# carlobaldassi/GaussDCA.jl

Measured on AMD Instinct MI355X. Metric: end-to-end gDCA sec + achieved Cholesky TFLOP/s, N=500 M=50k q=21, higher is better.
Workload: dtype f64

## Files before the change

gaussdca.jl_amd/csrc/gdca_hamming_form.h:

```cpp
#pragma once

#if defined(__HIPCC__)
#define GDCA_FORM_HD __host__ __device__
#else
#define GDCA_FORM_HD
#endif

#define HAM_CAND_PER_TILE 64
#define HAM_FORM_MAX_DENSITY (0.5 * HAM_CAND_PER_TILE / 16384.0)

#define HAM_FORM_BOUND3_DENSITY 1e-3

#define HAM_T_DENSE 1.9e-3
#define HAM_CUT_TAIL 0.35
#define HAM_T_PAIR 0.7e-4
#define HAM_T_REFINE 1.3e-7
#define HAM_T_TILE 6.5e-3
#define HAM_T_ENTRY 1.6e-4
#define HAM_T_IMAGE 4.0e-5
#define HAM_T_FIXED 25.0

#define HAM_FORM_MIN_WORK 65536.0

static inline GDCA_FORM_HD double gdca_hamming_tiles(int M)
{
    const double Mt = (double)((M + 127) / 128);
    return 0.5 * Mt * (Mt + 1.0);
}

static inline GDCA_FORM_HD int gdca_hamming_consensus_gate(int N, int M)
{
    const int NW = (N + 31) / 32;
    return NW > 2 && gdca_hamming_tiles(M) * (double)NW >= HAM_FORM_MIN_WORK;
}

static inline GDCA_FORM_HD int gdca_hamming_pick_form(double cand3, double cand1, double pairs, int N, int M, int cut)
{
    if (!(pairs > 0.0)) return 0;
    const int NW = (N + 31) / 32;
    const double tiles = gdca_hamming_tiles(M), all = 0.5 * (double)M * (double)M;
    const double f3 = cand3 / pairs, f1 = cand1 / pairs;
    const int other = f3 < HAM_FORM_BOUND3_DENSITY ? 1 : 0;
    if (cand1 < 0.0 || f1 > HAM_FORM_MAX_DENSITY) return other;
    const double weff = (cut > 0 && cut < NW) ? (double)cut + HAM_CUT_TAIL * (double)(NW - cut) : (double)NW;
    const double E = (double)((NW + 7) / 8 * 8), pair = HAM_T_PAIR + (double)N * HAM_T_REFINE;
    const double cost_other = other ? tiles * weff * HAM_T_DENSE + f3 * all * pair : tiles * (double)NW * 1.5 * HAM_T_DENSE;
    const double cost_cons = tiles * (HAM_T_TILE + E * HAM_T_ENTRY) + f1 * all * pair + (double)M * E * HAM_T_IMAGE + HAM_T_FIXED;
    return cost_cons < cost_other ? 2 : other;
}
```

gaussdca.jl_amd/csrc/k_hamming_fp4.hip:

```cpp
#include <algorithm>

#include "gdca_internal.h"
#include "gdca_launch.h"

typedef int fp4x8_t __attribute__((ext_vector_type(8)));
typedef float f32x16_t __attribute__((ext_vector_type(16)));

#define F4_TILE 256
#define F4_KC 4
#define F4_ROW (F4_KC * 32 + 16)
#define F4_OP (F4_TILE * F4_ROW)
#define F4_LDS (4 * F4_OP)
#define F4_SEG 8

static inline int f4_entries(int NW) { return (NW + 2 * F4_KC - 1) / (2 * F4_KC) * (2 * F4_KC); }
static inline size_t f4_image_only_bytes(int N, int M)
{
    const size_t NW = (size_t)(N + 31) / 32, rows = ((size_t)M + F4_TILE - 1) / F4_TILE * F4_TILE;
    return rows * (size_t)f4_entries((int)NW) * 16;
}
size_t gdca_fp4_image_bytes(int N, int M)
{
    return f4_image_only_bytes(N, M) + (size_t)f4_entries((N + 31) / 32) * 32;
}

__device__ __forceinline__ uint32_t f4_spread8(uint32_t b)
{
    uint32_t x = b & 0xffu;
    x = (x | (x << 12)) & 0x000f000fu;
    x = (x | (x << 6)) & 0x03030303u;
    x = (x | (x << 3)) & 0x11111111u;
    return x;
}
__device__ __forceinline__ uint32_t f4_nibbles8(uint32_t differs, uint32_t valid)
{
    return ((f4_spread8(differs) << 3) | 0x22222222u) & (f4_spread8(valid) * 0xfu);
}
__device__ __forceinline__ uint32_t f4_signs8(uint32_t v)
{
    uint32_t x = (v >> 3) & 0x11111111u;
    x = (x | (x >> 3)) & 0x03030303u;
    x = (x | (x >> 6)) & 0x000f000fu;
    x = (x | (x >> 12)) & 0xffu;
    return x;
}

struct k_fp4_sigma_args {
    const uint32_t *hist;
    uint8_t *sigma;
    int N, NP;
};
template <int CAP>
__global__ __launch_bounds__(256) void k_fp4_sigma(const BatchArgs<k_fp4_sigma_args, CAP> B_)
{
    GDCA_MEMBER(B_);
    const uint32_t *__restrict__ hist = a_.hist;
    const int i = blockIdx.x * 256 + threadIdx.x;
    if (i >= a_.NP) return;
    uint32_t best = 0u, bz = 0u;
    if (i < a_.N) {
        const uint4 *h = reinterpret_cast<const uint4 *>(hist + (size_t)i * 32);
#pragma unroll
        for (int g = 0; g < 8; ++g) {
            const uint4 v = h[g];
            const uint32_t c[4] = {v.x, v.y, v.z, v.w};
#pragma unroll
// ... 16 lines not shown
template <int CAP>
__global__ __launch_bounds__(256) void k_fp4_image(const BatchArgs<k_fp4_image_args, CAP> B_)
{
    GDCA_MEMBER(B_);
    const int8_t *__restrict__ Z = a_.Z;
    const uint8_t *__restrict__ sigma = a_.sigma;
    uint4 *__restrict__ img = a_.img;
    const int N = a_.N, M = a_.M, E = a_.E;
    const long long g = (long long)blockIdx.x * 256 + threadIdx.x;
    if (g >= (long long)a_.rows * E) return;
    const int k = (int)(g / E), w = (int)(g - (long long)k * E);
    uint32_t diff = 0u, valid = 0u;
    const int nb = min(32, N - w * 32);
    if (k < M && nb > 0) {
        const int8_t *src = Z + (size_t)k * N + (size_t)w * 32;
        valid = nb == 32 ? 0xffffffffu : ((1u << nb) - 1u);
        if (nb == 32 && (N & 3) == 0 && (reinterpret_cast<uintptr_t>(Z) & 3) == 0) {
            const uint32_t *s4 = reinterpret_cast<const uint32_t *>(src), *g4 = reinterpret_cast<const uint32_t *>(sigma + w * 32);
#pragma unroll
            for (int j = 0; j < 8; ++j) {
                uint32_t x = (s4[j] & 0x1f1f1f1fu) ^ g4[j];
                x |= x >> 4;
                x |= x >> 2;
                x |= x >> 1;
                x &= 0x01010101u;
                diff |= (((x * 0x01020408u) >> 24) & 0xfu) << (4 * j);
            }
        } else {
            for (int b = 0; b < nb; ++b) diff |= (uint32_t)(((uint32_t)(uint8_t)src[b] & 31u) != (uint32_t)sigma[w * 32 + b]) << b;
        }
    }
    img[g] = make_uint4(f4_nibbles8(diff, valid), f4_nibbles8(diff >> 8, valid >> 8), f4_nibbles8(diff >> 16, valid >> 16), f4_nibbles8(diff >> 24, valid >> 24));
}

__device__ __forceinline__ void f4_tri_decode(int t, int Mt, int &I, int &J)
{
    const double b = 2.0 * Mt + 1.0;
    int i = (int)((b - sqrt(b * b - 8.0 * (double)t)) * 0.5);
    i = max(0, min(i, Mt - 1));
    auto start = [Mt](int r) { return (long long)r * Mt - (long long)r * (r - 1) / 2; };
    while (i > 0 && start(i) > t) --i;
    while (i < Mt - 1 && start(i + 1) <= t) ++i;
    I = i;
    J = i + (int)(t - start(i));
}

struct k_hamming_fp4_args {
    const unsigned char *img;
    int E, M, Mt, N;
    gdca_dev_scalars *sc;
    int2 *cand_list;
    unsigned cand_cap;
};
__shared__ unsigned f4_tile_n[2], f4_tile_base;
template <int CAP, bool ARES>
__global__ __launch_bounds__(1024) void k_hamming_fp4(const BatchArgs<k_hamming_fp4_args, CAP> B_)
{
    GDCA_MEMBER(B_);
    gdca_dev_scalars *__restrict__ sc = a_.sc;
    if (sc->ham_mode != 2) return;
    const int thresh = sc->thresh;
    if (thresh <= 0) return;
    const unsigned char *__restrict__ img = a_.img;
    const int E = a_.E, M = a_.M, Mt = a_.Mt;
    int2 *__restrict__ cand_list = a_.cand_list;
    const unsigned cand_cap = a_.cand_cap;
    extern __shared__ __attribute__((aligned(16))) unsigned char f4_lds[];

    const int I = (int)blockIdx.y, J0 = I + (int)blockIdx.x * F4_SEG;
    if (J0 >= Mt) return;
    const int J1 = min(Mt, J0 + F4_SEG);
    const int tid = threadIdx.x, lane = tid & 63, wv = tid >> 6, wr = wv & 3, wc = wv >> 2;
    const int l32 = lane & 31, lh = lane >> 5;
    if (tid == 0) {
        f4_tile_n[0] = 0u;
        f4_tile_n[1] = 0u;
    }
    const size_t rowbytes = (size_t)E * 16;
    const int nchunk = E / (2 * F4_KC);
    const int total = (J1 - J0) * nchunk;

    const int srow = tid >> 3, spc = tid & 7;
    const unsigned char *ga = img + ((size_t)I * F4_TILE + srow) * rowbytes + spc * 16;
    const unsigned char *gb0 = img + (size_t)srow * rowbytes + spc * 16;
    const size_t half = (size_t)128 * rowbytes, tilebytes = (size_t)F4_TILE * rowbytes;
    unsigned char *la = f4_lds + srow * F4_ROW + spc * 16;
    uint4 s0, s1, s2, s3;
    s0 = s1 = make_uint4(0u, 0u, 0u, 0u);
#define F4_LOAD_A(ch)                                                                     \
    do {                                                                                  \
        s0 = *reinterpret_cast<const uint4 *>(ga + (size_t)(ch) * (32 * F4_KC));          \
        s1 = *reinterpret_cast<const uint4 *>(ga + half + (size_t)(ch) * (32 * F4_KC));   \
    } while (0)
#define F4_LOAD_B(J, ch)                                                                                      \
    do {                                                                                                      \
        const unsigned char *g_ = gb0 + (size_t)(J) * tilebytes + (size_t)(ch) * (32 * F4_KC);                \
        s2 = *reinterpret_cast<const uint4 *>(g_);                                                            \
        s3 = *reinterpret_cast<const uint4 *>(g_ + half);                                                     \
    } while (0)
#define F4_STORE_A(region)                                                                \
    do {                                                                                  \
        unsigned char *d_ = la + (size_t)(region) * F4_OP;                                \
        *reinterpret_cast<uint4 *>(d_) = s0;                                              \
        *reinterpret_cast<uint4 *>(d_ + 128 * F4_ROW) = s1;                               \
    } while (0)
#define F4_STORE_B(buf)                                                                   \
    do {                                                                                  \
        unsigned char *d_ = la + (size_t)(2 + (buf)) * F4_OP;                             \
        *reinterpret_cast<uint4 *>(d_) = s2;                                              \
        *reinterpret_cast<uint4 *>(d_ + 128 * F4_ROW) = s3;                               \
    } while (0)

    f32x16_t acc[2][2];
#pragma unroll
    for (int i = 0; i < 2; ++i)
#pragma unroll
        for (int j = 0; j < 2; ++j)
#pragma unroll
            for (int e = 0; e < 16; ++e) acc[i][j][e] = 0.f;
    const int one = 0x7f7f7f7f;

    const unsigned char *abase = f4_lds + (wr * 64 + l32) * F4_ROW + lh * 16, *bbase = f4_lds + 2 * F4_OP + (wc * 64 + l32) * F4_ROW + lh * 16;
    const float limit = (float)(a_.N - 2 * thresh);

    if constexpr (ARES) {
        F4_LOAD_A(0);
        F4_STORE_A(0);
        if (nchunk > 1) {
            F4_LOAD_A(1);
            F4_STORE_A(1);
        }
    } else {
        F4_LOAD_A(0);
        F4_STORE_A(0);
    }
    F4_LOAD_B(J0, 0);
    F4_STORE_B(0);
    __syncthreads();
    int J = J0, ch = 0;
    for (int it = 0; it < total; ++it) {
        const int buf = it & 1;
        const bool more = it + 1 < total;
        const bool last = ch + 1 == nchunk;
        const int Jn = last ? J + 1 : J, chn = last ? 0 : ch + 1;
        if (more) {
            if constexpr (!ARES) F4_LOAD_A(chn);
            F4_LOAD_B(Jn, chn);
        }
        const unsigned char *As = abase + (size_t)(ARES ? ch : buf) * F4_OP, *Bs = bbase + (size_t)buf * F4_OP;
#pragma unroll 1
        for (int ks = 0; ks < F4_KC; ++ks) {
            fp4x8_t a[2], b[2];
#pragma unroll
            for (int i = 0; i < 2; ++i) {
                const uint4 x = *reinterpret_cast<const uint4 *>(As + i * 32 * F4_ROW + ks * 32);
                a[i] = (fp4x8_t){(int)x.x, (int)x.y, (int)x.z, (int)x.w, 0, 0, 0, 0};
            }
#pragma unroll
            for (int j = 0; j < 2; ++j) {
                const uint4 x = *reinterpret_cast<const uint4 *>(Bs + j * 32 * F4_ROW + ks * 32);
                b[j] = (fp4x8_t){(int)x.x, (int)x.y, (int)x.z, (int)x.w, 0, 0, 0, 0};
            }
#pragma unroll
            for (int i = 0; i < 2; ++i)
#pragma unroll
                for (int j = 0; j < 2; ++j)
                    acc[i][j] = __builtin_amdgcn_mfma_scale_f32_32x32x64_f8f6f4(a[i], b[j], acc[i][j], 4, 4, 0, one, 0, one);
        }
        if (more) {
            if constexpr (!ARES) F4_STORE_A(buf ^ 1);
            F4_STORE_B(buf ^ 1);
        }
        if (last) {
            const int slot_n = (J - J0) & 1;
            const bool diag = I == J;
            unsigned mine = 0;
            unsigned long long cand[2] = {0ull, 0ull};
            float mx = acc[0][0][0];
#pragma unroll
            for (int i = 0; i < 2; ++i)
#pragma unroll
                for (int j = 0; j < 2; ++j)
#pragma unroll
                    for (int e = 0; e < 16; ++e) mx = fmaxf(mx, acc[i][j][e]);
            if (mx > limit) {
#pragma unroll
                for (int i = 0; i < 2; ++i)
#pragma unroll
                    for (int j = 0; j < 2; ++j) {
                        const int gc = J * F4_TILE + wc * 64 + j * 32 + l32;
#pragma unroll
                        for (int e = 0; e < 16; ++e) {
                            const int gr = I * F4_TILE + wr * 64 + i * 32 + 8 * (e >> 2) + 4 * lh + (e & 3);
                            if (acc[i][j][e] > limit && gr < M && gc < M && (diag ? gr < gc : true)) {
                                cand[i] |= 1ull << (16 * j + e);
                                ++mine;
                            }
                        }
                    }
            }
#pragma unroll
            for (int i = 0; i < 2; ++i)
#pragma unroll
                for (int j = 0; j < 2; ++j)
#pragma unroll
                    for (int e = 0; e < 16; ++e) acc[i][j][e] = 0.f;
            const unsigned off = mine ? atomicAdd(&f4_tile_n[slot_n], mine) : 0u;
            __syncthreads();
            const unsigned ntile = f4_tile_n[slot_n];
            if (tid == 0) f4_tile_n[slot_n ^ 1] = 0u;
            if (ntile != 0u) {
                if (tid == 0) {
                    const unsigned long long base = atomicAdd(&sc->ham_ncand, (unsigned long long)ntile);
                    f4_tile_base = base > (unsigned long long)cand_cap ? cand_cap : (unsigned)base;
                }
                __syncthreads();
                unsigned slot = f4_tile_base + off;
#pragma unroll
                for (int i = 0; i < 2; ++i) {
                    unsigned long long c = cand[i];
                    while (c) {
                        const int bit = __builtin_ctzll(c), j = bit >> 4, e = bit & 15;
                        const int gr = I * F4_TILE + wr * 64 + i * 32 + 8 * (e >> 2) + 4 * lh + (e & 3);
                        const int gc = J * F4_TILE + wc * 64 + j * 32 + l32;
                        if (slot < cand_cap) cand_list[slot] = make_int2(gr, gc);
                        ++slot;
                        c &= c - 1;
                    }
                }
            }
        }
        J = Jn;
        ch = chn;
        __syncthreads();
    }
}

#define F4_PW 8
struct k_fp4_probe_args {
    const uint4 *img;
    int E, NW, M, Mt;
    gdca_dev_scalars *sc;
};
template <int CAP>
__global__ __launch_bounds__(256) void k_fp4_probe(const BatchArgs<k_fp4_probe_args, CAP> B_)
{
    GDCA_MEMBER(B_);
    const uint4 *__restrict__ img = a_.img;
    const int E = a_.E, NW = a_.NW, M = a_.M, Mt = a_.Mt;
    gdca_dev_scalars *sc = a_.sc;
    const int thresh = sc->thresh;
    if (thresh <= 0) return;
    __shared__ int total;
    __shared__ uint32_t bits[2][F4_PW][128];
    int I, J;
    f4_tri_decode((int)(((long long)blockIdx.x * ((long long)Mt * (Mt + 1) / 2)) / gridDim.x), Mt, I, J);
    const int tid = threadIdx.x, tx = tid & 15, ty = tid >> 4;
    if (tid == 0) total = 0;
    int D[8][8];
#pragma unroll
    for (int r = 0; r < 8; ++r)
#pragma unroll
        for (int c = 0; c < 8; ++c) D[r][c] = 0;
    const uint4 *mine = img + (size_t)((tid < 128 ? I : J) * 128 + (tid & 127)) * E;
    for (int w0 = 0; w0 < NW; w0 += F4_PW) {
        __syncthreads();
#pragma unroll
        for (int u = 0; u < F4_PW; ++u) {
            uint32_t b = 0u;
            if (w0 + u < NW) {
                const uint4 v = mine[w0 + u];
                b = f4_signs8(v.x) | (f4_signs8(v.y) << 8) | (f4_signs8(v.z) << 16) | (f4_signs8(v.w) << 24);
            }
            bits[tid >> 7][u][tid & 127] = b;
        }
        __syncthreads();
        const int wn = min(F4_PW, NW - w0);
        for (int u = 0; u < wn; ++u) {
            uint32_t a[8], b[8];
#pragma unroll
            for (int r = 0; r < 8; ++r) a[r] = bits[0][u][ty * 8 + r];
#pragma unroll
            for (int c = 0; c < 8; ++c) b[c] = bits[1][u][tx * 8 + c];
#pragma unroll
            for (int r = 0; r < 8; ++r)
#pragma unroll
                for (int c = 0; c < 8; ++c) D[r][c] += __builtin_popcount(a[r] ^ b[c]);
        }
    }
    int cand = 0;
#pragma unroll
    for (int r = 0; r < 8; ++r)
#pragma unroll
        for (int c = 0; c < 8; ++c) {
            const int gr = I * 128 + ty * 8 + r, gc = J * 128 + tx * 8 + c;
            cand += (gr < M) && (gc < M) && (gr != gc) && (D[r][c] < thresh);
        }
    if (cand) atomicAdd(&total, cand);
    __syncthreads();
    if (tid == 0 && total) atomicAdd(&sc->ham_cand2, total);
}

void gdca_launch_hamming_fp4_image(hipStream_t s, const int8_t *Z, const uint32_t *hist, void *img, int N, int M)
{
    const int NW = (N + 31) / 32, E = f4_entries(NW), rows = (M + F4_TILE - 1) / F4_TILE * F4_TILE;
    uint8_t *sigma = (uint8_t *)img + f4_image_only_bytes(N, M);
    gdca_launch<k_fp4_sigma_args, k_fp4_sigma<1>, k_fp4_sigma<GDCA_MAXB>>(dim3((unsigned)((32 * E + 255) / 256)), dim3(256), 0, s, k_fp4_sigma_args{hist, sigma, N, 32 * E});
    const long long items = (long long)rows * E;
    gdca_launch<k_fp4_image_args, k_fp4_image<1>, k_fp4_image<GDCA_MAXB>>(dim3((unsigned)((items + 255) / 256)), dim3(256), 0, s,
                                                                           k_fp4_image_args{Z, sigma, (uint4 *)img, N, M, E, rows});
}

void gdca_launch_hamming_fp4_probe(hipStream_t s, const void *img, int N, int M, int nprobe, gdca_dev_scalars *sc)
{
    const int NW = (N + 31) / 32, Mt = (M + 127) / 128;
    gdca_launch<k_fp4_probe_args, k_fp4_probe<1>, k_fp4_probe<GDCA_MAXB>>(dim3((unsigned)nprobe), dim3(256), 0, s,
                                                                           k_fp4_probe_args{(const uint4 *)img, f4_entries(NW), NW, M, Mt, sc});
}

void gdca_launch_hamming_fp4(hipStream_t s, const void *img, int N, int M, gdca_dev_scalars *sc, void *cand_list, unsigned cap)
{
    const int NW = (N + 31) / 32, E = f4_entries(NW), Mt = (M + F4_TILE - 1) / F4_TILE;
    const dim3 grid((unsigned)((Mt + F4_SEG - 1) / F4_SEG), (unsigned)Mt);
    const k_hamming_fp4_args a{(const unsigned char *)img, E, M, Mt, N, sc, (int2 *)cand_list, cap};
    if (E <= 4 * F4_KC)
        gdca_launch<k_hamming_fp4_args, k_hamming_fp4<1, true>, k_hamming_fp4<GDCA_MAXB, true>>(grid, dim3(1024), F4_LDS, s, a);
    else
        gdca_launch<k_hamming_fp4_args, k_hamming_fp4<1, false>, k_hamming_fp4<GDCA_MAXB, false>>(grid, dim3(1024), F4_LDS, s, a);
}
```

gaussdca.jl_amd/csrc/k_tally.hip:

```cpp
#include "gdca_internal.h"
#include "gdca_launch.h"
#include <cstdlib>

typedef unsigned long long u64;

#define PIK_THREADS 512
#define PIK_SLABS 4
struct k_pi_keep_args {
    const int8_t *Zt;
    const u64 *Wfix;
    u64 *Pifix;
    uint32_t *keep;
    int *keep_n;
    uint8_t *sigma;
    int N;
    int M;
    int q;
    gdca_dev_scalars *sc;
};
static inline k_pi_keep_args k_pi_keep_mk(const int8_t *Zt, const u64 *Wfix, u64 *Pifix, uint32_t *keep, int *keep_n, uint8_t *sigma, int N, int M, int q, gdca_dev_scalars *sc)
{
    return k_pi_keep_args{Zt, Wfix, Pifix, keep, keep_n, sigma, N, M, q, sc};
}
template <int CAP>
// ... 258 lines not shown
void gdca_launch_pi_finalize(hipStream_t s, const u64 *Pifix, int N, int q, int fix_shift, const double *Meff_dev,
                             double pc, double *Pi_true, double *Pi_pc, double *pi_max)
{
    const int n = N * (q - 1);
    (gdca_launch<k_pi_finalize_args, k_pi_finalize<1>, k_pi_finalize<GDCA_MAXB>>(dim3((n + 255) / 256), dim3(256), 0, s, k_pi_finalize_mk(Pifix, N, q, fix_shift, Meff_dev, pc, Pi_true, Pi_pc, pi_max)));
}

#define TALLY_THREADS 1024
#define TALLY_CHUNK 1024

struct k_pair_tally_args {
    const int8_t *Zc;
    const int8_t *Zt;
    const u64 *Wfix;
    int N;
    int M;
    int q;
    int fix_shift;
    const double *Meff_dev;
    double pc;
    const double *Pi_pc;
    int mode;
    double *out;
    size_t ld;
    const uint32_t *keep;
    const int *keep_n;
    const uint8_t *sigma;
    const u64 *Pifix;
};
static inline k_pair_tally_args k_pair_tally_mk(const int8_t *Zc, const int8_t *Zt, const u64 *Wfix, int N, int M, int q, int fix_shift, const double *Meff_dev, double pc, const double *Pi_pc, int mode, double *out, size_t ld,
                                                const uint32_t *keep, const int *keep_n, const uint8_t *sigma, const u64 *Pifix)
{
    return k_pair_tally_args{Zc, Zt, Wfix, N, M, q, fix_shift, Meff_dev, pc, Pi_pc, mode, out, ld, keep, keep_n, sigma, Pifix};
}
template <int CAP, int TJ, bool SKIP>
__global__ __launch_bounds__(TALLY_THREADS) void k_pair_tally(const BatchArgs<k_pair_tally_args, CAP> B_)
{
    GDCA_MEMBER(B_);
    const int8_t *__restrict__ Zc = a_.Zc;
    const int8_t *__restrict__ Zt = a_.Zt;
    const u64 *__restrict__ Wfix = a_.Wfix;
    int N = a_.N;
    int M = a_.M;
    int q = a_.q;
    int fix_shift = a_.fix_shift;
    const double *__restrict__ Meff_dev = a_.Meff_dev;
    double pc = a_.pc;
    const double *__restrict__ Pi_pc = a_.Pi_pc;
    int mode = a_.mode;
    double *__restrict__ out = a_.out;
    size_t ld = a_.ld;
    extern __shared__ __attribute__((aligned(16))) unsigned char smem[];
    const int s = q - 1;
    const int i = blockIdx.y;
    const int jblk = (blockIdx.x + blockIdx.y) % gridDim.x;
    const int j0 = jblk * TJ;
    if (j0 + TJ - 1 < i) return;

    const int NROW = SKIP ? q : s;
    const int CB = SKIP ? 0 : 1;
    const int RS = (SKIP ? q : s + 2) * TJ;
    u64 *hist = reinterpret_cast<u64 *>(smem);
    u64 *meta_s = hist + (size_t)NROW * RS;
    uint8_t *zs = reinterpret_cast<uint8_t *>(meta_s + TALLY_CHUNK);

    const int tid = threadIdx.x, lane = tid & 63, wv = tid >> 6;
    constexpr int SPI = 64 / TJ;
    constexpr int NWAVE = TALLY_THREADS / 64;
    constexpr int SEQ_PER_WAVE = TALLY_CHUNK / NWAVE;
    constexpr int NV = TJ / 16;
    static_assert(TALLY_CHUNK == TALLY_THREADS, "one staged sequence per thread");
    const int jl = lane % TJ, sub = lane / TJ;
    const u64 wmask = (1ull << 59) - 1;
    const unsigned qclamp = (unsigned)(SKIP ? q - 1 : s + 1);
    const int nk = SKIP ? a_.keep_n[i] : M;
    const uint32_t *__restrict__ keep_i = a_.keep + (size_t)i * M;

    for (int e = tid; e < NROW * RS; e += TALLY_THREADS) hist[e] = 0;

    const int8_t *Zblk = Zc + (size_t)jblk * M * TJ;
    uint4 z0 = make_uint4(0, 0, 0, 0), z1 = z0;
    u64 wf = 0;
    int8_t av = 0;
#define TALLY_FETCH(KC)                                                                       \
    do {                                                                                      \
        int k_ = (KC) + tid;                                                                  \
        k_ = k_ < nk ? k_ : nk - 1;              \
        if (SKIP) {                                                                           \
            const uint32_t e_ = keep_i[k_];                                                   \
            av = (int8_t)(e_ & 31u);                                                          \
            k_ = (int)(e_ >> 5);                                                              \
        }                                                                                     \
        const uint4 *src_ = reinterpret_cast<const uint4 *>(Zblk + (size_t)k_ * TJ);          \
        z0 = src_[0];                                                                         \
        if (NV > 1) z1 = src_[1];                                                             \
        if (!SKIP) av = Zt[(size_t)i * M + k_];                                               \
        wf = Wfix[k_];                                                                        \
    } while (0)
    if (nk > 0) TALLY_FETCH(0);
    for (int kc = 0; kc < nk; kc += TALLY_CHUNK) {
        __syncthreads();
        {
            reinterpret_cast<uint4 *>(zs + (size_t)tid * TJ)[0] = z0;
            if (NV > 1) reinterpret_cast<uint4 *>(zs + (size_t)tid * TJ)[1] = z1;
            const unsigned a = (unsigned)(uint8_t)av - 1u;
            const bool valid = (SKIP || a < (unsigned)s) && (kc + tid < nk);
            meta_s[tid] = valid ? (((u64)a << 59) | (wf & wmask)) : 0ull;
        }
        __syncthreads();
        if (kc + TALLY_CHUNK < nk) TALLY_FETCH(kc + TALLY_CHUNK);
        const int kw = wv * SEQ_PER_WAVE;
#pragma unroll 2
        for (int it = 0; it < SEQ_PER_WAVE / SPI; it += 4) {
            u64 m4[4];
            unsigned b4[4];
#pragma unroll
            for (int u = 0; u < 4; ++u) {
                const int kk = kw + (it + u) * SPI + sub;
                m4[u] = meta_s[kk];
                b4[u] = zs[kk * TJ + jl];
            }
#pragma unroll
            for (int u = 0; u < 4; ++u) {
                const unsigned a = (unsigned)(m4[u] >> 59);
                const unsigned b = min(b4[u] - (unsigned)(1 - CB), qclamp);
                const unsigned idx = __umul24(a, (unsigned)RS) + __umul24(b, (unsigned)TJ) + (unsigned)jl;
                atomicAdd(&hist[idx], m4[u] & wmask);
            }
        }
    }
    __syncthreads();
#undef TALLY_FETCH

    if (SKIP) {
        const int sg = (int)a_.sigma[i] - 1;
        const u64 *__restrict__ Pifix = a_.Pifix;
        if (sg < s) {
            for (int e = tid; e < s * TJ; e += TALLY_THREADS) {
                const int b = e / TJ, l = e - b * TJ;
                const int jj = j0 + l;
                if (jj >= N || jj < i) continue;
                u64 v = Pifix[(size_t)jj * 32 + b + 1];
                for (int a = 0; a < q; ++a)
                    if (a != sg) v -= hist[(size_t)a * RS + b * TJ + l];
                hist[(size_t)sg * RS + b * TJ + l] = v;
            }
        }
    }

    double *pi_i = reinterpret_cast<double *>(meta_s);
    double *pi_j = pi_i + 32;
    if (mode == 1) {
        for (int e = tid; e < s; e += TALLY_THREADS) pi_i[e] = Pi_pc[i * s + e];
        for (int e = tid; e < TJ * s; e += TALLY_THREADS) {
            const int jj = j0 + e / s;
            pi_j[e] = (jj < N) ? Pi_pc[jj * s + (e % s)] : 0.0;
        }
    }
    __syncthreads();
    const double Meff = *Meff_dev;
    const double pcq = pc / (double)q;
    const double off_add = pcq / (double)q;
    const int total = s * s * TJ;
    for (int e = tid; e < total; e += TALLY_THREADS) {
        const int a = e / (TJ * s), rem = e - a * (TJ * s);
        const int l = rem / s, b = rem - l * s;
        const int jj = j0 + l;
        if (jj >= N || jj < i) continue;
        const double pt = ldexp((double)hist[(size_t)a * RS + (b + CB) * TJ + l], -fix_shift) / Meff;
        double v = pt;
        if (mode == 1) {
            const double pij = (jj != i) ? ((1.0 - pc) * pt + off_add) : ((1.0 - pc) * pt + ((a == b) ? pcq : 0.0));
            v = pij - pi_i[a] * pi_j[rem];
        }
        out[(size_t)(jj * s + b) + (size_t)(i * s + a) * ld] = v;
    }
    for (int e = tid; e < total; e += TALLY_THREADS) {
        const int l = e / (s * s), rem = e - l * (s * s);
        const int b = rem / s, a = rem - b * s;
        const int jj = j0 + l;
        if (jj >= N || jj <= i) continue;
        const double pt = ldexp((double)hist[(size_t)a * RS + (b + CB) * TJ + l], -fix_shift) / Meff;
        double v = pt;
        if (mode == 1) {
            const double pij = (1.0 - pc) * pt + off_add;
            v = pij - pi_i[a] * pi_j[l * s + b];
        }
        out[(size_t)(i * s + a) + (size_t)(jj * s + b) * ld] = v;
    }
}

static size_t tally_lds_bytes(int s, int TJ, bool skip = false)
{
    const size_t hist = skip ? (size_t)(s + 1) * (s + 1) * TJ * 8 : (size_t)s * (s + 2) * TJ * 8;
    return hist + (size_t)TALLY_CHUNK * 8 + (size_t)TALLY_CHUNK * TJ;
}

int gdca_tally_tj(int q, int tj_wanted)
{
    if (tj_wanted == 32 && tally_lds_bytes(q - 1, 32) <= 160 * 1024) return 32;
    return 16;
}

bool gdca_tally_skip(int q, int TJ, int skip_wanted, int M)
{
    const size_t lds = 160 * 1024, full = tally_lds_bytes(q - 1, TJ), skip = tally_lds_bytes(q - 1, TJ, true);
    return skip_wanted && M <= (1 << 27) && skip <= lds && lds / skip >= lds / full;
}

void gdca_launch_pair_tally(hipStream_t st, const int8_t *Zc, const int8_t *Zt, const u64 *Wfix, int N, int M, int q,
                            int fix_shift, const double *Meff_dev, double pc, const double *Pi_pc, int mode,
                            double *out, size_t ld, int TJ, const uint32_t *keep, const int *keep_n, const uint8_t *sigma,
                            const u64 *Pifix)
{
    const int s = q - 1;
    const bool skip = keep != nullptr;
    const k_pair_tally_args a = k_pair_tally_mk(Zc, Zt, Wfix, N, M, q, fix_shift, Meff_dev, pc, Pi_pc, mode, out, ld, keep, keep_n, sigma, Pifix);
    const size_t lds = tally_lds_bytes(s, TJ, skip);
    if (TJ == 32) {
        if (skip)
            (gdca_launch<k_pair_tally_args, k_pair_tally<1, 32, true>, k_pair_tally<GDCA_MAXB, 32, true>>(dim3((N + 31) / 32, N), dim3(TALLY_THREADS), lds, st, a));
        else
            (gdca_launch<k_pair_tally_args, k_pair_tally<1, 32, false>, k_pair_tally<GDCA_MAXB, 32, false>>(dim3((N + 31) / 32, N), dim3(TALLY_THREADS), lds, st, a));
    } else {
        if (skip)
            (gdca_launch<k_pair_tally_args, k_pair_tally<1, 16, true>, k_pair_tally<GDCA_MAXB, 16, true>>(dim3((N + 15) / 16, N), dim3(TALLY_THREADS), lds, st, a));
        else
            (gdca_launch<k_pair_tally_args, k_pair_tally<1, 16, false>, k_pair_tally<GDCA_MAXB, 16, false>>(dim3((N + 15) / 16, N), dim3(TALLY_THREADS), lds, st, a));
    }
}

#define COV_ROWS_PER_THREAD 4
struct k_cov_from_pij_args {
    const double *Pij;
    const double *Pi_pc;
    int n;
    int q;
    double pc;
    double *out;
    size_t ld;
};
static inline k_cov_from_pij_args k_cov_from_pij_mk(const double *Pij, const double *Pi_pc, int n, int q, double pc, double *out, size_t ld)
{
    return k_cov_from_pij_args{Pij, Pi_pc, n, q, pc, out, ld};
}
template <int CAP>
__global__ __launch_bounds__(256) void k_cov_from_pij(const BatchArgs<k_cov_from_pij_args, CAP> B_)
{
    GDCA_MEMBER(B_);
    const double *__restrict__ Pij = a_.Pij;
    const double *__restrict__ Pi_pc = a_.Pi_pc;
    int n = a_.n;
    int q = a_.q;
    double pc = a_.pc;
    double *__restrict__ out = a_.out;
    size_t ld = a_.ld;
    const int s = q - 1;
    const int c = blockIdx.y;
    const int ic = c / s;
    const double pcq = pc / (double)q;
    const double off_add = pcq / (double)q;
    const double pi_c = Pi_pc[c];
    const double *__restrict__ src = Pij + (size_t)c * n;
    double *__restrict__ dst = out + (size_t)c * ld;
    const int r0 = blockIdx.x * (256 * COV_ROWS_PER_THREAD) + threadIdx.x;
    double pt[COV_ROWS_PER_THREAD], pr[COV_ROWS_PER_THREAD];
#pragma unroll
    for (int u = 0; u < COV_ROWS_PER_THREAD; ++u) {
        const int r = r0 + u * 256;
        pt[u] = r < n ? src[r] : 0.0;
        pr[u] = r < n ? Pi_pc[r] : 0.0;
    }
#pragma unroll
    for (int u = 0; u < COV_ROWS_PER_THREAD; ++u) {
        const int r = r0 + u * 256;
        if (r >= n) continue;
        const int jj = r / s, i = ic;
        const bool ab = r == c;
        const double pij = (jj != i) ? ((1.0 - pc) * pt[u] + off_add) : ((1.0 - pc) * pt[u] + (ab ? pcq : 0.0));
        dst[r] = pij - pi_c * pr[u];
    }
// ... 9 lines not shown
```

Baseline: 52.41.

## Restructure FP4 Hamming MFMA kernel: 512 threads, wider warp tiles, deeper pipelined loads

Rewrites the FP4 Hamming candidate kernel to use 512-thread blocks where each wave computes a 64x128 tile (2x4 MFMA accumulators). It loads through buffer resources, prefetches two chunks ahead, and schedules LDS reads against MFMAs with sched_group_barrier. It also remaps the grid to a 1D triangular walk enumeration with XCD-aware interleaving and defers candidate writes by one tile to overlap the global atomic. The cost-model constants for the consensus form are lowered to match, so the form picker will choose this path more often. This raises register pressure and adds complexity in the triple-buffered tile counters and the deferred-write synchronisation.

```diff
diff --git a/gaussdca.jl_amd/csrc/gdca_hamming_form.h b/gaussdca.jl_amd/csrc/gdca_hamming_form.h
--- a/gaussdca.jl_amd/csrc/gdca_hamming_form.h
+++ b/gaussdca.jl_amd/csrc/gdca_hamming_form.h
@@ -15,8 +15,8 @@
 #define HAM_CUT_TAIL 0.35
 #define HAM_T_PAIR 0.7e-4
 #define HAM_T_REFINE 1.3e-7
-#define HAM_T_TILE 6.5e-3
-#define HAM_T_ENTRY 1.6e-4
+#define HAM_T_TILE 4.8e-3
+#define HAM_T_ENTRY 1.2e-4
 #define HAM_T_IMAGE 4.0e-5
 #define HAM_T_FIXED 25.0
 
diff --git a/gaussdca.jl_amd/csrc/k_hamming_fp4.hip b/gaussdca.jl_amd/csrc/k_hamming_fp4.hip
--- a/gaussdca.jl_amd/csrc/k_hamming_fp4.hip
+++ b/gaussdca.jl_amd/csrc/k_hamming_fp4.hip
@@ -5,6 +5,8 @@
 
 typedef int fp4x8_t __attribute__((ext_vector_type(8)));
 typedef float f32x16_t __attribute__((ext_vector_type(16)));
+typedef unsigned u32x4_t __attribute__((ext_vector_type(4)));
+typedef float f32x2_t __attribute__((ext_vector_type(2)));
 
 #define F4_TILE 256
 #define F4_KC 4
@@ -12,6 +14,7 @@
 #define F4_OP (F4_TILE * F4_ROW)
 #define F4_LDS (4 * F4_OP)
 #define F4_SEG 8
+#define F4_THREADS 512
 
 static inline int f4_entries(int NW) { return (NW + 2 * F4_KC - 1) / (2 * F4_KC) * (2 * F4_KC); }
 static inline size_t f4_image_only_bytes(int N, int M)
@@ -134,9 +137,138 @@
     int2 *cand_list;
     unsigned cand_cap;
 };
-__shared__ unsigned f4_tile_n[2], f4_tile_base;
+__shared__ unsigned f4_tile_n[3], f4_tile_base;
+
+static inline __host__ __device__ unsigned f4_walks(int Mt)
+{
+    const unsigned nb = (unsigned)((Mt + F4_SEG - 1) / F4_SEG);
+    return (F4_SEG / 2) * (nb - 1) * nb + (unsigned)Mt;
+}
+
+__device__ __forceinline__ fp4x8_t f4_frag(const unsigned char *p)
+{
+    const uint4 x = *reinterpret_cast<const uint4 *>(p);
+    return (fp4x8_t){(int)x.x, (int)x.y, (int)x.z, (int)x.w, 0, 0, 0, 0};
+}
+template <bool FIRST, bool TWOSETS>
+__device__ __forceinline__ void f4_chunk(f32x16_t (&acc)[2][4], const unsigned char *As, const unsigned char *Bs)
+{
+    static_assert(F4_KC == 4, "the schedule below is written for four k steps");
+    const int one = 0x7f7f7f7f;
+    const f32x16_t zero = (f32x16_t)(0.f);
+    fp4x8_t a0[2], b0[4], a1[2], b1[4];
+    (void)a1, (void)b1;
+#define F4_READ(a, b, ks)                                                        \
+    do {                                                                         \
+        _Pragma("unroll") for (int i = 0; i < 2; ++i) a[i] = f4_frag(As + i * 32 * F4_ROW + (ks) * 32); \
+        _Pragma("unroll") for (int j = 0; j < 4; ++j) b[j] = f4_frag(Bs + j * 32 * F4_ROW + (ks) * 32); \
+    } while (0)
+#define F4_MUL(a, b, C)                                                          \
+    do {                                                                         \
+        _Pragma("unroll") for (int i = 0; i < 2; ++i)                            \
+            _Pragma("unroll") for (int j = 0; j < 4; ++j)                        \
+                acc[i][j] = __builtin_amdgcn_mfma_scale_f32_32x32x64_f8f6f4(a[i], b[j], C, 4, 4, 0, one, 0, one); \
+    } while (0)
+    if constexpr (TWOSETS) {
+        F4_READ(a0, b0, 0);
+        F4_READ(a1, b1, 1);
+        if constexpr (FIRST)
+            F4_MUL(a0, b0, zero);
+        else
+            F4_MUL(a0, b0, acc[i][j]);
+        F4_READ(a0, b0, 2);
+        F4_MUL(a1, b1, acc[i][j]);
+        F4_READ(a1, b1, 3);
+        F4_MUL(a0, b0, acc[i][j]);
+        F4_MUL(a1, b1, acc[i][j]);
+        __builtin_amdgcn_sched_group_barrier(0x100, 6, 0);
+#pragma unroll
+        for (int ks = 0; ks + 1 < F4_KC; ++ks)
+#pragma unroll
+            for (int m = 0; m < 8; ++m) {
+                __builtin_amdgcn_sched_group_barrier(0x008, 1, 0);
+                if (m < 6) __builtin_amdgcn_sched_group_barrier(0x100, 1, 0);
+            }
+        __builtin_amdgcn_sched_group_barrier(0x008, 8, 0);
+    } else {
+        F4_READ(a0, b0, 0);
+        if constexpr (FIRST)
+            F4_MUL(a0, b0, zero);
+        else
+            F4_MUL(a0, b0, acc[i][j]);
+#pragma unroll 1
+        for (int ks = 1; ks < F4_KC; ++ks) {
+            F4_READ(a0, b0, ks);
+            F4_MUL(a0, b0, acc[i][j]);
+        }
+    }
+#undef F4_READ
+#undef F4_MUL
+}
+
+__device__ __forceinline__ void f4_tile_candidates(const f32x16_t (&acc)[2][4], const float limit, const int I, const int J, const int M, const int wr,
+                                                   const int wc, const int l32, const int lh, const int slot_n, unsigned long long (&cand)[2],
+                                                   unsigned &off)
+{
+    unsigned mine = 0u;
+    cand[0] = cand[1] = 0ull;
+    const bool diag = I == J, edge = diag || (J + 1) * F4_TILE > M;
+    int rb = I * F4_TILE + wr * 64 + 4 * lh, cb = J * F4_TILE + wc * 128 + l32;
+    asm volatile("" : "+v"(rb), "+v"(cb));
+#pragma unroll
+    for (int i = 0; i < 2; ++i)
+#pragma unroll
+        for (int j = 0; j < 4; ++j) {
+            float mx = acc[i][j][0];
+#pragma unroll
+            for (int e = 1; e < 16; ++e) mx = __builtin_amdgcn_fmed3f(mx, acc[i][j][e], __builtin_inff());
+            if (mx > limit) {
+                unsigned m16 = 0u;
+#pragma unroll
+                for (int e = 14; e >= 0; e -= 2) {
+                    const f32x2_t d = (f32x2_t)(limit) - (f32x2_t){acc[i][j][e], acc[i][j][e + 1]};
+                    m16 = __builtin_amdgcn_alignbit(m16, __float_as_uint(d.y), 31u);
+                    m16 = __builtin_amdgcn_alignbit(m16, __float_as_uint(d.x), 31u);
+                }
+                if (edge) {
+                    const int gc = cb + j * 32;
+#pragma unroll
+                    for (int e = 0; e < 16; ++e) {
+                        const int gr = rb + i * 32 + 8 * (e >> 2) + (e & 3);
+                        if (!(gr < M && gc < M && (diag ? gr < gc : true))) m16 &= ~(1u << e);
+                    }
+                }
+                cand[i] |= (unsigned long long)m16 << (16 * j);
+                mine += (unsigned)__builtin_popcount(m16);
+            }
+        }
+    off = mine ? atomicAdd(&f4_tile_n[slot_n], mine) : 0u;
+}
+__device__ __forceinline__ unsigned f4_tile_count(const int tid, const int slot_n)
+{
+    const unsigned ntile = f4_tile_n[slot_n];
+    if (tid == 0) f4_tile_n[slot_n == 0 ? 2 : slot_n - 1] = 0u;
+    return (unsigned)__builtin_amdgcn_readfirstlane((int)ntile);
+}
+__device__ __forceinline__ void f4_tile_write(int2 *cand_list, const unsigned cand_cap, const int I, const int J, const int wr, const int wc, const int l32,
+                                              const int lh, const unsigned long long (&cand)[2], unsigned slot)
+{
+#pragma unroll
+    for (int i = 0; i < 2; ++i) {
+        unsigned long long c = cand[i];
+        while (c) {
+            const int bit = __builtin_ctzll(c), j = bit >> 4, e = bit & 15;
+            const int gr = I * F4_TILE + wr * 64 + i * 32 + 8 * (e >> 2) + 4 * lh + (e & 3);
+            const int gc = J * F4_TILE + wc * 128 + j * 32 + l32;
+            if (slot < cand_cap) cand_list[slot] = make_int2(gr, gc);
+            ++slot;
+            c &= c - 1;
+        }
+    }
+}
+
 template <int CAP, bool ARES>
-__global__ __launch_bounds__(1024) void k_hamming_fp4(const BatchArgs<k_hamming_fp4_args, CAP> B_)
+__global__ __launch_bounds__(F4_THREADS) void k_hamming_fp4(const BatchArgs<k_hamming_fp4_args, CAP> B_)
 {
     GDCA_MEMBER(B_);
     gdca_dev_scalars *__restrict__ sc = a_.sc;
@@ -149,173 +281,170 @@
     const unsigned cand_cap = a_.cand_cap;
     extern __shared__ __attribute__((aligned(16))) unsigned char f4_lds[];
 
-    const int I = (int)blockIdx.y, J0 = I + (int)blockIdx.x * F4_SEG;
-    if (J0 >= Mt) return;
-    const int J1 = min(Mt, J0 + F4_SEG);
+    int I, J0, J1;
+    {
+        const unsigned id = blockIdx.x, x = id & 7u, k = id >> 3;
+        const unsigned v = ((k >> 5) * 8u + x) * 32u + (k & 31u);
+        if (v >= f4_walks(Mt)) return;
+        int c = (int)((sqrtf((float)v + 1.f) - 1.f) * 0.5f);
+        c = max(c, 0);
+        while (c > 0 && (unsigned)((F4_SEG / 2) * c * (c + 1)) > v) --c;
+        while ((unsigned)((F4_SEG / 2) * (c + 1) * (c + 2)) <= v) ++c;
+        I = (int)(v - (unsigned)((F4_SEG / 2) * c * (c + 1)));
+        J0 = max(I, c * F4_SEG);
+        J1 = min(Mt, (c + 1) * F4_SEG);
+    }
+    if (I >= Mt || J0 >= J1) return;
     const int tid = threadIdx.x, lane = tid & 63, wv = tid >> 6, wr = wv & 3, wc = wv >> 2;
     const int l32 = lane & 31, lh = lane >> 5;
     if (tid == 0) {
         f4_tile_n[0] = 0u;
         f4_tile_n[1] = 0u;
+        f4_tile_n[2] = 0u;
     }
     const size_t rowbytes = (size_t)E * 16;
     const int nchunk = E / (2 * F4_KC);
     const int total = (J1 - J0) * nchunk;
 
     const int srow = tid >> 3, spc = tid & 7;
-    const unsigned char *ga = img + ((size_t)I * F4_TILE + srow) * rowbytes + spc * 16;
-    const unsigned char *gb0 = img + (size_t)srow * rowbytes + spc * 16;
-    const size_t half = (size_t)128 * rowbytes, tilebytes = (size_t)F4_TILE * rowbytes;
-    unsigned char *la = f4_lds + srow * F4_ROW + spc * 16;
-    uint4 s0, s1, s2, s3;
-    s0 = s1 = make_uint4(0u, 0u, 0u, 0u);
-#define F4_LOAD_A(ch)                                                                     \
-    do {                                                                                  \
-        s0 = *reinterpret_cast<const uint4 *>(ga + (size_t)(ch) * (32 * F4_KC));          \
-        s1 = *reinterpret_cast<const uint4 *>(ga + half + (size_t)(ch) * (32 * F4_KC));   \
+    const unsigned voff = (unsigned)srow * (unsigned)rowbytes + (unsigned)spc * 16u, quarter = 64u * (unsigned)rowbytes;
+    const size_t tilebytes = (size_t)F4_TILE * rowbytes;
+    const unsigned char *ga = img + (size_t)I * tilebytes;
+    const unsigned char *gn = img + (size_t)J0 * tilebytes;
+    int ldch = 0;
+    unsigned char *la = f4_lds + srow * F4_ROW + spc * 16, *lb = la + 2 * F4_OP;
+#define F4_LOAD(S, g, live)                                                                                                \
+    do {                                                                                                                \
+        const __amdgpu_buffer_rsrc_t r_ = __builtin_amdgcn_make_buffer_rsrc(const_cast<unsigned char *>(g), 0, (live) ? (int)tilebytes : 0, 0x00020000); \
+        S##0 = __builtin_amdgcn_raw_buffer_load_b128(r_, (int)voff, 0, 0);                                              \
+        S##1 = __builtin_amdgcn_raw_buffer_load_b128(r_, (int)voff, (int)quarter, 0);                                   \
+        S##2 = __builtin_amdgcn_raw_buffer_load_b128(r_, (int)voff, (int)(2u * quarter), 0);                            \
+        S##3 = __builtin_amdgcn_raw_buffer_load_b128(r_, (int)voff, (int)(3u * quarter), 0);                            \
     } while (0)
-#define F4_LOAD_B(J, ch)                                                                                      \
-    do {                                                                                                      \
-        const unsigned char *g_ = gb0 + (size_t)(J) * tilebytes + (size_t)(ch) * (32 * F4_KC);                \
-        s2 = *reinterpret_cast<const uint4 *>(g_);                                                            \
-        s3 = *reinterpret_cast<const uint4 *>(g_ + half);                                                     \
+#define F4_STORE(S, l, region)                                            \
+    do {                                                                  \
+        unsigned char *d_ = (l) + (region) * F4_OP;                       \
+        *reinterpret_cast<u32x4_t *>(d_) = S##0;                          \
+        *reinterpret_cast<u32x4_t *>(d_ + 64 * F4_ROW) = S##1;            \
+        *reinterpret_cast<u32x4_t *>(d_ + 128 * F4_ROW) = S##2;           \
+        *reinterpret_cast<u32x4_t *>(d_ + 192 * F4_ROW) = S##3;           \
     } while (0)
-#define F4_STORE_A(region)                                                                \
-    do {                                                                                  \
-        unsigned char *d_ = la + (size_t)(region) * F4_OP;                                \
-        *reinterpret_cast<uint4 *>(d_) = s0;                                              \
-        *reinterpret_cast<uint4 *>(d_ + 128 * F4_ROW) = s1;                               \
+#define F4_NEXT()                                                         \
+    do {                                                                  \
+        gn += 32 * F4_KC;                                                 \
+        if (++ldch == nchunk) {                                           \
+            ldch = 0;                                                     \
+            gn += tilebytes - (size_t)nchunk * (32 * F4_KC);              \
+        }                                                                 \
     } while (0)
-#define F4_STORE_B(buf)                                                                   \
-    do {                                                                                  \
-        unsigned char *d_ = la + (size_t)(2 + (buf)) * F4_OP;                             \
-        *reinterpret_cast<uint4 *>(d_) = s2;                                              \
-        *reinterpret_cast<uint4 *>(d_ + 128 * F4_ROW) = s3;                               \
-    } while (0)
-
-    f32x16_t acc[2][2];
-#pragma unroll
-    for (int i = 0; i < 2; ++i)
-#pragma unroll
-        for (int j = 0; j < 2; ++j)
-#pragma unroll
-            for (int e = 0; e < 16; ++e) acc[i][j][e] = 0.f;
-    const int one = 0x7f7f7f7f;
-
-    const unsigned char *abase = f4_lds + (wr * 64 + l32) * F4_ROW + lh * 16, *bbase = f4_lds + 2 * F4_OP + (wc * 64 + l32) * F4_ROW + lh * 16;
+    u32x4_t p0, p1, p2, p3, q0, q1, q2, q3;
+
+    const unsigned char *abase = f4_lds + (wr * 64 + l32) * F4_ROW + lh * 16, *bbase = f4_lds + 2 * F4_OP + (wc * 128 + l32) * F4_ROW + lh * 16;
     const float limit = (float)(a_.N - 2 * thresh);
 
     if constexpr (ARES) {
-        F4_LOAD_A(0);
-        F4_STORE_A(0);
-        if (nchunk > 1) {
-            F4_LOAD_A(1);
-            F4_STORE_A(1);
-        }
+        u32x4_t t0, t1, t2, t3, u0, u1, u2, u3;
+        F4_LOAD(t, ga, true);
+        F4_LOAD(u, ga + 32 * F4_KC, nchunk > 1);
+        F4_LOAD(p, gn, true);
+        F4_NEXT();
+        F4_LOAD(q, gn, total > 1);
+        if (total > 1) F4_NEXT();
+        F4_STORE(t, la, 0);
+        if (nchunk > 1) F4_STORE(u, la, 1);
+        F4_STORE(p, lb, 0);
+        F4_LOAD(p, gn, total > 2);
+        if (total > 2) F4_NEXT();
     } else {
-        F4_LOAD_A(0);
-        F4_STORE_A(0);
-    }
-    F4_LOAD_B(J0, 0);
-    F4_STORE_B(0);
+        u32x4_t t0, t1, t2, t3, u0, u1, u2, u3;
+        F4_LOAD(t, ga, true);
+        F4_LOAD(u, gn, true);
+        F4_NEXT();
+        F4_LOAD(p, ga + (size_t)ldch * (32 * F4_KC), total > 1);
+        F4_LOAD(q, gn, total > 1);
+        if (total > 1) F4_NEXT();
+        F4_STORE(t, la, 0);
+        F4_STORE(u, lb, 0);
+    }
+    f32x16_t acc[2][4];
     __syncthreads();
-    int J = J0, ch = 0;
-    for (int it = 0; it < total; ++it) {
-        const int buf = it & 1;
-        const bool more = it + 1 < total;
-        const bool last = ch + 1 == nchunk;
-        const int Jn = last ? J + 1 : J, chn = last ? 0 : ch + 1;
-        if (more) {
-            if constexpr (!ARES) F4_LOAD_A(chn);
-            F4_LOAD_B(Jn, chn);
-        }
-        const unsigned char *As = abase + (size_t)(ARES ? ch : buf) * F4_OP, *Bs = bbase + (size_t)buf * F4_OP;
-#pragma unroll 1
-        for (int ks = 0; ks < F4_KC; ++ks) {
-            fp4x8_t a[2], b[2];
-#pragma unroll
-            for (int i = 0; i < 2; ++i) {
-                const uint4 x = *reinterpret_cast<const uint4 *>(As + i * 32 * F4_ROW + ks * 32);
-                a[i] = (fp4x8_t){(int)x.x, (int)x.y, (int)x.z, (int)x.w, 0, 0, 0, 0};
-            }
-#pragma unroll
-            for (int j = 0; j < 2; ++j) {
-                const uint4 x = *reinterpret_cast<const uint4 *>(Bs + j * 32 * F4_ROW + ks * 32);
-                b[j] = (fp4x8_t){(int)x.x, (int)x.y, (int)x.z, (int)x.w, 0, 0, 0, 0};
-            }
-#pragma unroll
-            for (int i = 0; i < 2; ++i)
-#pragma unroll
-                for (int j = 0; j < 2; ++j)
-                    acc[i][j] = __builtin_amdgcn_mfma_scale_f32_32x32x64_f8f6f4(a[i], b[j], acc[i][j], 4, 4, 0, one, 0, one);
-        }
-        if (more) {
-            if constexpr (!ARES) F4_STORE_A(buf ^ 1);
-            F4_STORE_B(buf ^ 1);
-        }
-        if (last) {
-            const int slot_n = (J - J0) & 1;
-            const bool diag = I == J;
-            unsigned mine = 0;
-            unsigned long long cand[2] = {0ull, 0ull};
-            float mx = acc[0][0][0];
-#pragma unroll
-            for (int i = 0; i < 2; ++i)
-#pragma unroll
-                for (int j = 0; j < 2; ++j)
-#pragma unroll
-                    for (int e = 0; e < 16; ++e) mx = fmaxf(mx, acc[i][j][e]);
-            if (mx > limit) {
-#pragma unroll
-                for (int i = 0; i < 2; ++i)
-#pragma unroll
-                    for (int j = 0; j < 2; ++j) {
-                        const int gc = J * F4_TILE + wc * 64 + j * 32 + l32;
-#pragma unroll
-                        for (int e = 0; e < 16; ++e) {
-                            const int gr = I * F4_TILE + wr * 64 + i * 32 + 8 * (e >> 2) + 4 * lh + (e & 3);
-                            if (acc[i][j][e] > limit && gr < M && gc < M && (diag ? gr < gc : true)) {
-                                cand[i] |= 1ull << (16 * j + e);
-                                ++mine;
-                            }
-                        }
-                    }
-            }
-#pragma unroll
-            for (int i = 0; i < 2; ++i)
-#pragma unroll
-                for (int j = 0; j < 2; ++j)
-#pragma unroll
-                    for (int e = 0; e < 16; ++e) acc[i][j][e] = 0.f;
-            const unsigned off = mine ? atomicAdd(&f4_tile_n[slot_n], mine) : 0u;
-            __syncthreads();
-            const unsigned ntile = f4_tile_n[slot_n];
-            if (tid == 0) f4_tile_n[slot_n ^ 1] = 0u;
-            if (ntile != 0u) {
-                if (tid == 0) {
-                    const unsigned long long base = atomicAdd(&sc->ham_ncand, (unsigned long long)ntile);
-                    f4_tile_base = base > (unsigned long long)cand_cap ? cand_cap : (unsigned)base;
-                }
-                __syncthreads();
-                unsigned slot = f4_tile_base + off;
-#pragma unroll
-                for (int i = 0; i < 2; ++i) {
-                    unsigned long long c = cand[i];
-                    while (c) {
-                        const int bit = __builtin_ctzll(c), j = bit >> 4, e = bit & 15;
-                        const int gr = I * F4_TILE + wr * 64 + i * 32 + 8 * (e >> 2) + 4 * lh + (e & 3);
-                        const int gc = J * F4_TILE + wc * 64 + j * 32 + l32;
-                        if (slot < cand_cap) cand_list[slot] = make_int2(gr, gc);
-                        ++slot;
-                        c &= c - 1;
-                    }
-                }
-            }
-        }
-        J = Jn;
-        ch = chn;
+
+    int J = J0, ch = 0, slot_n = 0;
+    unsigned long long cand[2] = {0ull, 0ull};
+    unsigned off = 0u;
+    bool pend = false;
+    int pendJ = 0;
+    unsigned long long pbase = 0ull;
+    unsigned nowhere = 0u;
+    asm volatile("" : "+v"(nowhere));
+    unsigned long long *ncand_p = &sc->ham_ncand + nowhere;
+#define F4_ITER(PAR, SN, IT)                                                                                                    \
+    {                                                                                                                             \
+        const bool last = ch + 1 == nchunk;                                                                      \
+        if (ch == 0)                                                                                                              \
+            f4_chunk<true, ARES>(acc, abase + (size_t)(ARES ? ch : (PAR)) * F4_OP, bbase + (size_t)(PAR) * F4_OP);                      \
+        else                                                                                                                      \
+            f4_chunk<false, ARES>(acc, abase + (size_t)(ARES ? ch : (PAR)) * F4_OP, bbase + (size_t)(PAR) * F4_OP);                     \
+        if constexpr (ARES) {                                                                                                     \
+            if ((IT) + 1 < total) F4_STORE(SN, lb, (PAR) ^ 1);                                                                      \
+            F4_LOAD(SN, gn, (IT) + 3 < total);                                                                                      \
+            if ((IT) + 3 < total) F4_NEXT();                                                                                        \
+        } else {                                                                                                                  \
+            if ((IT) + 1 < total) {                                                                                                 \
+                F4_STORE(p, la, (PAR) ^ 1);                                                                                       \
+                F4_STORE(q, lb, (PAR) ^ 1);                                                                                       \
+            }                                                                                                                     \
+             \
+            __builtin_amdgcn_sched_barrier(0);                                                                                    \
+            F4_LOAD(p, ga + (size_t)ldch * (32 * F4_KC), (IT) + 2 < total);                                                         \
+            F4_LOAD(q, gn, (IT) + 2 < total);                                                                                       \
+            if ((IT) + 2 < total) F4_NEXT();                                                                                        \
+        }                                                                                                                         \
+        if (last) f4_tile_candidates(acc, limit, I, J, M, wr, wc, l32, lh, slot_n, cand, off);                                    \
+        if (pend && tid == 0) f4_tile_base = pbase > (unsigned long long)cand_cap ? cand_cap : (unsigned)pbase;                   \
+        __syncthreads();                                                                                                          \
+        if (pend) {                                                                                                               \
+            f4_tile_write(cand_list, cand_cap, I, pendJ, wr, wc, l32, lh, cand, f4_tile_base + off);                              \
+            pend = false;                                                                                                         \
+        }                                                                                                                         \
+        if (last) {                                                                                                               \
+            const unsigned ntile = f4_tile_count(tid, slot_n);                                                                    \
+            if (ntile != 0u) {                                                                                                    \
+                if (tid == 0) pbase = atomicAdd(ncand_p, (unsigned long long)ntile);                                              \
+                if (nchunk > 1) {                                                                                                 \
+                    pend = true;                                                                                                  \
+                    pendJ = J;                                                                                                    \
+                } else {                                                                                                          \
+                    if (tid == 0) f4_tile_base = pbase > (unsigned long long)cand_cap ? cand_cap : (unsigned)pbase;               \
+                    __syncthreads();                                                                                              \
+                    f4_tile_write(cand_list, cand_cap, I, J, wr, wc, l32, lh, cand, f4_tile_base + off);                          \
+                }                                                                                                                 \
+            }                                                                                                                     \
+            slot_n = slot_n == 2 ? 0 : slot_n + 1;                                                                                \
+            ++J;                                                                                                                  \
+            ch = 0;                                                                                                               \
+        } else                                                                                                                    \
+            ++ch;                                                                                                                 \
+    }
+    if constexpr (ARES) {
+        int it = 0;
+        for (; it + 1 < total; it += 2) {
+            F4_ITER(0, q, it)
+            F4_ITER(1, p, it + 1)
+        }
+        if (it < total) F4_ITER(0, q, it)
+    } else {
+        for (int it = 0; it < total; ++it) F4_ITER(it & 1, p, it)
+    }
+    if (pend) {
+        if (tid == 0) f4_tile_base = pbase > (unsigned long long)cand_cap ? cand_cap : (unsigned)pbase;
         __syncthreads();
-    }
+        f4_tile_write(cand_list, cand_cap, I, pendJ, wr, wc, l32, lh, cand, f4_tile_base + off);
+    }
+#undef F4_ITER
+#undef F4_LOAD
+#undef F4_STORE
+#undef F4_NEXT
 }
 
 #define F4_PW 8
@@ -403,10 +532,10 @@
 void gdca_launch_hamming_fp4(hipStream_t s, const void *img, int N, int M, gdca_dev_scalars *sc, void *cand_list, unsigned cap)
 {
     const int NW = (N + 31) / 32, E = f4_entries(NW), Mt = (M + F4_TILE - 1) / F4_TILE;
-    const dim3 grid((unsigned)((Mt + F4_SEG - 1) / F4_SEG), (unsigned)Mt);
+    const dim3 grid((f4_walks(Mt) + 255u) / 256u * 256u, 1u);
     const k_hamming_fp4_args a{(const unsigned char *)img, E, M, Mt, N, sc, (int2 *)cand_list, cap};
     if (E <= 4 * F4_KC)
-        gdca_launch<k_hamming_fp4_args, k_hamming_fp4<1, true>, k_hamming_fp4<GDCA_MAXB, true>>(grid, dim3(1024), F4_LDS, s, a);
+        gdca_launch<k_hamming_fp4_args, k_hamming_fp4<1, true>, k_hamming_fp4<GDCA_MAXB, true>>(grid, dim3(F4_THREADS), F4_LDS, s, a);
     else
-        gdca_launch<k_hamming_fp4_args, k_hamming_fp4<1, false>, k_hamming_fp4<GDCA_MAXB, false>>(grid, dim3(1024), F4_LDS, s, a);
-}
+        gdca_launch<k_hamming_fp4_args, k_hamming_fp4<1, false>, k_hamming_fp4<GDCA_MAXB, false>>(grid, dim3(F4_THREADS), F4_LDS, s, a);
+}
```

After: 53.25 (median of 6 runs). +1.6%, better.

## Launch only upper-triangle tally blocks, prefetch keep entries, trim tail iterations

Applied to the files above, without the earlier changes.

Replaces the 2D grid with a 1D grid that enumerates only (i, jblk) pairs on or above the diagonal. Block coordinates are recovered with a sqrt-based triangular inverse, launched in reverse order so the heaviest blocks start first. The keep-list entry is now loaded one chunk ahead, removing a dependent load from the fetch path. Each wave also limits its inner loop to the sequences remaining in the last chunk. This cuts launch of blocks that exit immediately and shortens the tail work, at the cost of a small per-block index computation and a float-sqrt rounding correction loop.

```diff
diff --git a/gaussdca.jl_amd/csrc/k_tally.hip b/gaussdca.jl_amd/csrc/k_tally.hip
--- a/gaussdca.jl_amd/csrc/k_tally.hip
+++ b/gaussdca.jl_amd/csrc/k_tally.hip
@@ -334,10 +334,21 @@
     size_t ld = a_.ld;
     extern __shared__ __attribute__((aligned(16))) unsigned char smem[];
     const int s = q - 1;
+#ifdef GDCA_TALLY_OLD_MAP
     const int i = blockIdx.y;
     const int jblk = (blockIdx.x + blockIdx.y) % gridDim.x;
     const int j0 = jblk * TJ;
     if (j0 + TJ - 1 < i) return;
+#else
+    const unsigned lin = gridDim.x * gridDim.y - 1u - (blockIdx.y * gridDim.x + blockIdx.x);
+    const unsigned tri = lin / TJ;
+    unsigned jb = (unsigned)((sqrtf(8.0f * (float)tri + 1.0f) - 1.0f) * 0.5f);
+    while (jb * (jb + 1u) / 2u > tri) --jb;
+    while ((jb + 1u) * (jb + 2u) / 2u <= tri) ++jb;
+    const int jblk = (int)jb;
+    const int j0 = jblk * TJ;
+    const int i = (int)(lin - (unsigned)TJ * (jb * (jb + 1u) / 2u));
+#endif
 
     const int NROW = SKIP ? q : s;
     const int CB = SKIP ? 0 : 1;
@@ -364,14 +375,21 @@
     uint4 z0 = make_uint4(0, 0, 0, 0), z1 = z0;
     u64 wf = 0;
     int8_t av = 0;
+    uint32_t en = 0;
+#define TALLY_ENTRY(KC)                                                                       \
+    do {                                                                                      \
+        if (SKIP) {                                                                           \
+            int k_ = (KC) + tid;                                                              \
+            en = keep_i[k_ < nk ? k_ : nk - 1];     \
+        }                                                                                     \
+    } while (0)
 #define TALLY_FETCH(KC)                                                                       \
     do {                                                                                      \
         int k_ = (KC) + tid;                                                                  \
         k_ = k_ < nk ? k_ : nk - 1;              \
         if (SKIP) {                                                                           \
-            const uint32_t e_ = keep_i[k_];                                                   \
-            av = (int8_t)(e_ & 31u);                                                          \
-            k_ = (int)(e_ >> 5);                                                              \
+            av = (int8_t)(en & 31u);                                                          \
+            k_ = (int)(en >> 5);                                                              \
         }                                                                                     \
         const uint4 *src_ = reinterpret_cast<const uint4 *>(Zblk + (size_t)k_ * TJ);          \
         z0 = src_[0];                                                                         \
@@ -379,7 +397,11 @@
         if (!SKIP) av = Zt[(size_t)i * M + k_];                                               \
         wf = Wfix[k_];                                                                        \
     } while (0)
-    if (nk > 0) TALLY_FETCH(0);
+    if (nk > 0) {
+        TALLY_ENTRY(0);
+        TALLY_FETCH(0);
+        TALLY_ENTRY(TALLY_CHUNK);
+    }
     for (int kc = 0; kc < nk; kc += TALLY_CHUNK) {
         __syncthreads();
         {
@@ -390,10 +412,15 @@
             meta_s[tid] = valid ? (((u64)a << 59) | (wf & wmask)) : 0ull;
         }
         __syncthreads();
-        if (kc + TALLY_CHUNK < nk) TALLY_FETCH(kc + TALLY_CHUNK);
+        if (kc + TALLY_CHUNK < nk) {
+            TALLY_FETCH(kc + TALLY_CHUNK);
+            TALLY_ENTRY(kc + 2 * TALLY_CHUNK);
+        }
         const int kw = wv * SEQ_PER_WAVE;
+        const int left = nk - kc - __builtin_amdgcn_readfirstlane(kw);
+        const int nit = left >= SEQ_PER_WAVE ? SEQ_PER_WAVE / SPI : left > 0 ? (left + 4 * SPI - 1) / (4 * SPI) * 4 : 0;
 #pragma unroll 2
-        for (int it = 0; it < SEQ_PER_WAVE / SPI; it += 4) {
+        for (int it = 0; it < nit; it += 4) {
             u64 m4[4];
             unsigned b4[4];
 #pragma unroll
@@ -478,6 +505,16 @@
     return hist + (size_t)TALLY_CHUNK * 8 + (size_t)TALLY_CHUNK * TJ;
 }
 
+static dim3 tally_grid(int N, int TJ)
+{
+#ifdef GDCA_TALLY_OLD_MAP
+    return dim3((N + TJ - 1) / TJ, N);
+#else
+    const unsigned long long nblk = ((unsigned)N + TJ - 1) / TJ;
+    return dim3((unsigned)((unsigned long long)TJ * (nblk * (nblk - 1) / 2) + (unsigned)N), 1);
+#endif
+}
+
 int gdca_tally_tj(int q, int tj_wanted)
 {
     if (tj_wanted == 32 && tally_lds_bytes(q - 1, 32) <= 160 * 1024) return 32;
@@ -499,16 +536,17 @@
     const bool skip = keep != nullptr;
     const k_pair_tally_args a = k_pair_tally_mk(Zc, Zt, Wfix, N, M, q, fix_shift, Meff_dev, pc, Pi_pc, mode, out, ld, keep, keep_n, sigma, Pifix);
     const size_t lds = tally_lds_bytes(s, TJ, skip);
+    const dim3 grid = tally_grid(N, TJ);
     if (TJ == 32) {
         if (skip)
-            (gdca_launch<k_pair_tally_args, k_pair_tally<1, 32, true>, k_pair_tally<GDCA_MAXB, 32, true>>(dim3((N + 31) / 32, N), dim3(TALLY_THREADS), lds, st, a));
+            (gdca_launch<k_pair_tally_args, k_pair_tally<1, 32, true>, k_pair_tally<GDCA_MAXB, 32, true>>(grid, dim3(TALLY_THREADS), lds, st, a));
         else
-            (gdca_launch<k_pair_tally_args, k_pair_tally<1, 32, false>, k_pair_tally<GDCA_MAXB, 32, false>>(dim3((N + 31) / 32, N), dim3(TALLY_THREADS), lds, st, a));
+            (gdca_launch<k_pair_tally_args, k_pair_tally<1, 32, false>, k_pair_tally<GDCA_MAXB, 32, false>>(grid, dim3(TALLY_THREADS), lds, st, a));
     } else {
         if (skip)
-            (gdca_launch<k_pair_tally_args, k_pair_tally<1, 16, true>, k_pair_tally<GDCA_MAXB, 16, true>>(dim3((N + 15) / 16, N), dim3(TALLY_THREADS), lds, st, a));
+            (gdca_launch<k_pair_tally_args, k_pair_tally<1, 16, true>, k_pair_tally<GDCA_MAXB, 16, true>>(grid, dim3(TALLY_THREADS), lds, st, a));
         else
-            (gdca_launch<k_pair_tally_args, k_pair_tally<1, 16, false>, k_pair_tally<GDCA_MAXB, 16, false>>(dim3((N + 15) / 16, N), dim3(TALLY_THREADS), lds, st, a));
+            (gdca_launch<k_pair_tally_args, k_pair_tally<1, 16, false>, k_pair_tally<GDCA_MAXB, 16, false>>(grid, dim3(TALLY_THREADS), lds, st, a));
     }
 }
 
```

New measurement: 51.77 before, 52.34 after (median of 6 runs). +1.1%, better.
